# ucsdarclab/diffco

Measured on AMD Instinct MI355X. Metric: million collision-score+grad evals/sec, 7-DoF FK-kernel, 2k supports, higher is better.
Workload: dtype f32

## Files before the change

diffco_amd/csrc/score_kernel.h:

```cpp
#pragma once
#include <hip/hip_runtime.h>
#include <type_traits>
#include <stdint.h>
#include "fk_device.h"

namespace dcx {

enum { KF_RQ2 = 0,
       KF_POLY1 = 1,
       KF_GEN = 2 };

enum { MODE_SCORE = 0,
       MODE_GRAD_ROW = 1,
       MODE_GRAD_UP = 2 };

struct ScoreArgs {
    const float* rows;
    const float* centre;
    const FkProg* fk;
    const float* q;
    const float* upstream;
    float* score;
    float* grad;
    int64_t B;
// ... 117 lines not shown
#endif
#define DCX_D2_ACCS(D) (!DCX_D2_MULTI ? 1 : (D) >= 32 ? 4 : (D) >= 16 ? 2 : 1)
#ifndef DCX_PAIR2
#define DCX_PAIR2 1
#endif
#ifndef DCX_PAIR2_MAX_D
#define DCX_PAIR2_MAX_D 8
#endif
#ifndef DCX_PAIR2_LOADS
#define DCX_PAIR2_LOADS 1
#endif
#ifndef DCX_LOAD_GROUPS
#define DCX_LOAD_GROUPS 1
#endif

template <int KF, bool CLAMPED = false>
__device__ __forceinline__ void kernel_eval(float d2, const ScoreArgs& a, float& val, float& g) {
    if constexpr (KF == KF_RQ2) {
        const float t = fmaf(0.5f * a.kp0, d2, 1.0f);
        const float u = __builtin_amdgcn_rcpf(t);
        val = u * u;
        g = (-2.0f * a.kp0) * (val * u);
    } else if constexpr (KF == KF_POLY1) {
        const float d2c = CLAMPED ? d2 : fmaxf(d2, 1e-30f);
        const float ri = __builtin_amdgcn_rsqf(d2c);
        val = d2c * ri;
        g = ri;
    } else {
        if (a.kind == DCX_K_RQ) {
            const float p = a.kp1;
            const float t = fmaf(a.kp0 / p, d2, 1.0f);
            val = powf(t, -p);
            g = (-2.0f * a.kp0) * val * __builtin_amdgcn_rcpf(t);
        } else if (a.kind == DCX_K_POLY) {
            const int k = (int)a.kp0;
            const float ie = 1.0f / a.kp1;
            const float d2c = fmaxf(d2, 1e-30f);
            const float ri = __builtin_amdgcn_rsqf(d2c);
            const float r = d2c * ri;
            float rk2 = (k >= 2) ? 1.0f : ri;
            for (int i = 2; i < k; ++i) rk2 *= r;
            if (k & 1) {
                val = rk2 * d2c * ie;
                g = (float)k * rk2 * ie;
            } else {
                const float lg = 0.5f * logf(d2c);
                val = rk2 * d2c * lg * ie;
                g = rk2 * fmaf((float)k, lg, 1.0f) * ie;
            }
        } else {
            const float ie2 = 1.0f / (a.kp0 * a.kp0);
            const float v2 = fmaf(d2, ie2, 1.0f);
            const float rv = __builtin_amdgcn_rsqf(v2);
            val = v2 * rv;
            g = rv * ie2;
        }
    }
}

template <int KF>
__device__ __forceinline__ float d2_seed(const ScoreArgs& a) {
    if constexpr (KF == KF_RQ2) return a.kp0;
    else return 0.0f;
}
template <int KF>
inline constexpr float kGradScale = (KF == KF_RQ2) ? -4.0f : 1.0f;
template <int KF, bool CLAMPED = false>
__device__ __forceinline__ void sweep_eval(float t, const ScoreArgs& a, float& val, float& g) {
    if constexpr (KF == KF_RQ2) {
        const float u = __builtin_amdgcn_rcpf(t);
        val = u * u;
        g = val * u;
    } else {
        kernel_eval<KF, CLAMPED>(t, a, val, g);
    }
}

struct LdsPlan {
    int fk, q, x, g, f, red, total;
};
__host__ __device__ inline LdsPlan lds_plan(int dof, int d_fk, int frame_floats, int red_slots, int acc_floats,
                                            bool alias_xg = false) {
    LdsPlan p;
    p.x = 0;
    p.g = alias_xg ? p.x : p.x + 64 * d_fk;
    p.red = p.x;
    const int end_xg = p.g + 64 * d_fk;
    const int end_red = p.red + (red_slots < 1 ? 1 : red_slots) * acc_floats * 64;
    p.q = end_xg > end_red ? end_xg : end_red;
    p.f = p.q + ((64 * dof + 3) & ~3);
    p.fk = p.f + 64 * frame_floats;
    p.total = p.fk;
    return p;
}

#ifndef DCX_MINW_SLACK
#define DCX_MINW_SLACK 0
#endif
constexpr int sweep_min_waves(int D, int CC, int KF, bool QT = false) {
    if (QT) return 4;
    const int need = 3 * D + 2 * CC + 16 + DCX_MINW_SLACK + (KF == 2 ? 40 : 0);
    return need <= 64 ? 8 : need <= 72 ? 7 : need <= 80 ? 6 : need <= 96 ? 5 : need <= 128 ? 4 : need <= 168 ? 3 : need <= 256 ? 2 : 1;
}

__device__ __forceinline__ int fresh_lane() {
    int l = (int)__builtin_amdgcn_mbcnt_hi(~0u, __builtin_amdgcn_mbcnt_lo(~0u, 0u));
    asm volatile("" : "+v"(l));
    return l;
}

template <class Args>
__device__ __forceinline__ const __attribute__((address_space(4))) Args& reload_kernargs() {
    auto p = (const __attribute__((address_space(4))) Args*)__builtin_amdgcn_kernarg_segment_ptr();
    asm volatile("" : "+s"(p));
    return *p;
}
__device__ __forceinline__ const __attribute__((address_space(4))) ScoreArgs& reload_args() { return reload_kernargs<ScoreArgs>(); }
#define DCX_COPY_DH(dst, src)          \
    do {                               \
        (dst).prog = (src).prog;       \
        (dst).n_dwords = (src).n_dwords; \
        (dst).n_steps = (src).n_steps; \
        (dst).end0 = (src).end0;       \
        (dst).n_chains = (src).n_chains; \
        (dst).pt = (src).pt;           \
        (dst).bare = (src).bare;       \
        (dst).real = (src).real;       \
        (dst).n_pt = (src).n_pt;       \
        (dst).shared_q = (src).shared_q; \
    } while (0)

__device__ __forceinline__ void row_opaque(float& u, float& v) { asm volatile("" : "+v"(u), "+v"(v)); }

#ifndef DCX_XF_TAU
#define DCX_XF_TAU 0.01f
#endif
#ifndef DCX_XF_FLUSH
#define DCX_XF_FLUSH 64
#endif

constexpr bool xf_applies(int D, int CC, int KF) {
    const int used = D + CC + (CC > 1 ? 1 : 0);
    const int parts = (4 * used <= (CC > 1 ? DCX_P0_MAX_MULTI : DCX_P0_MAX_SINGLE)) ? 0 : (used + 37) / 38;
    return (KF == KF_POLY1 || KF == KF_RQ2) && used + 1 <= 38 && parts <= 1;
}
constexpr bool spare_applies(int D, int CC, int KF) {
    return CC == 1 && (D % 4) == 0 && D >= 4 && D <= 12 && (KF == KF_POLY1 || KF == KF_RQ2) && D + 4 <= (D + 2 + 3) / 4 * 4;
}
constexpr bool p2_applies(int D, int CC, int KF) {
    return DCX_PAIR2 && DCX_PAIR2_LOADS && CC == 1 && (D % 2) == 0 && D <= DCX_PAIR2_MAX_D && 4 * (D + 1) <= DCX_P0_MAX_SINGLE &&
           (KF == KF_RQ2 || KF == KF_POLY1);
}

template <int D, int KF, int CC, int MODE, bool XF = false, int NACC = 0, bool NS = false, bool SP = false>
__device__ __forceinline__ void sweep_rows(const ScoreArgs& a, const float (&x_in)[D], const float (&up)[CC], int j0, int j1,
                                           float (&sc)[CC], float (&gx)[D]) {
    static_assert(!NS || (CC > 1 && MODE == MODE_GRAD_UP), "NS: the gradient sweep of a multi-class model");
    static_assert(!SP || (XF && spare_applies(D, CC, KF) && xf_applies(D, CC, KF)), "the spare form: expanded, one class, D = 4, 8, 12");
    float x[D];
    float e_sp = 0.0f, tot_sp = 0.0f;
    int col_sp = 0;
    if constexpr (SP) {
        const int c = a.spare - 1;
        e_sp = x_in[D - 1];
#pragma unroll
        for (int k = 0; k + 1 < D; ++k) {
            e_sp = (k == c) ? x_in[k] : e_sp;
            x[k] = (k == c) ? x_in[D - 1] : x_in[k];
        }
        x[D - 1] = 0.0f;
        col_sp = c;
        asm volatile("" : "+v"(col_sp));
    } else {
#pragma unroll
        for (int k = 0; k < D; ++k) x[k] = x_in[k];
    }
    using L = RowLayout<D, CC>;
    constexpr bool GRAD = (MODE != MODE_SCORE);
    v2f gx2[D / 2 + 1];
#pragma unroll
    for (int k = 0; k < D / 2 + 1; ++k) gx2[k] = v2f{0.0f, 0.0f};
    cfloat_ptr rows = (cfloat_ptr)(uintptr_t)a.rows;
    if constexpr (SP) {
        uint64_t rp = (uint64_t)(uintptr_t)a.rows;
        asm volatile("" : "+s"(rp));
        rows = (cfloat_ptr)(uintptr_t)rp;
    }
    constexpr int USED_DIRECT = D + CC + (CC > 1 ? 1 : 0);
    constexpr bool XFA = XF && xf_applies(D, CC, KF);
    constexpr int USED = SP ? D + 4 : USED_DIRECT + (XFA ? 1 : 0);
    constexpr int RSTRIDE = L::RS;
    constexpr int PARTS = SP ? 0 : (4 * USED <= (CC > 1 ? DCX_P0_MAX_MULTI : DCX_P0_MAX_SINGLE)) ? 0 : (USED + 37) / 38;
    constexpr bool SC2 = (CC > 1 && PARTS == 1);
    v2f sc2[CC / 2 + 1];
#pragma unroll
    for (int i = 0; i < CC / 2 + 1; ++i) sc2[i] = v2f{0.0f, 0.0f};
    auto add_scores = [&](auto weight_of, float val) __attribute__((always_inline)) {
        if constexpr (NS) {
            (void)val;
        } else if constexpr (SC2) {
            const v2f v2 = {val, val};
#pragma unroll
            for (int c = 0; c + 1 < CC; c += 2) sc2[c / 2] = __builtin_elementwise_fma(v2f{weight_of(c), weight_of(c + 1)}, v2, sc2[c / 2]);
            if constexpr (CC & 1) sc[CC - 1] = fmaf(weight_of(CC - 1), val, sc[CC - 1]);
#pragma unroll
            for (int c = 0; c + 1 < CC; c += 2) asm volatile("" : "+v"(sc2[c / 2]));
            if constexpr (CC & 1) asm volatile("" : "+v"(sc[CC - 1]));
        } else {
#pragma unroll
            for (int c = 0; c < CC; ++c) sc[c] = fmaf(weight_of(c), val, sc[c]);
        }
    };

    v2f xm[D / 2 + 1], ga[D / 2 + 1];
    float xm_tail = 0.0f, ga_tail = 0.0f, xx = 0.0f, thr = 1e-30f, asum = 0.0f;
    if constexpr (XFA) {
#pragma unroll
        for (int k = 0; k < D; ++k) xx = fmaf(x[k], x[k], xx);
        if constexpr (SP) xx = fmaf(e_sp, e_sp, xx);
        thr = fmaxf(DCX_XF_TAU * xx, 1e-30f);
#pragma unroll
        for (int k = 0; k + 1 < D; k += 2) {
            xm[k / 2] = v2f{-2.0f * x[k], -2.0f * x[k + 1]};
            ga[k / 2] = v2f{0.0f, 0.0f};
        }
        if constexpr (D & 1) xm_tail = -2.0f * x[D - 1];
        if constexpr (SP) xm[D / 2 - 1].y = 1.0f;
    }
    auto d2_x = [&](const auto& r) __attribute__((always_inline)) -> float {
        constexpr int NA = NACC > 0 ? NACC : DCX_D2_ACCS(D);
        v2f acc[NA];
        if constexpr (SP) acc[0] = v2f{xx, 0.0f};
        else acc[0] = v2f{xx + r[L::SS_OFF], 0.0f};
#pragma unroll
        for (int i = 1; i < NA; ++i) acc[i] = v2f{0.0f, 0.0f};
#pragma unroll
        for (int k = 0; k + 1 < D; k += 2) {
            const v2f rv = {r[k], r[k + 1]};
            acc[(k / 2) % NA] = __builtin_elementwise_fma(xm[k / 2], rv, acc[(k / 2) % NA]);
        }
#pragma unroll
        for (int i = 1; i < NA; ++i) acc[0] += acc[i];
        float d2 = acc[0].x + acc[0].y;
        if constexpr (D & 1) d2 = fmaf(xm_tail, r[D - 1], d2);
        if constexpr (KF == KF_POLY1) return fmaxf(d2, thr);
        else return d2;
    };
    auto coef_of = [&](const auto& r, float g) __attribute__((always_inline)) -> float {
        if constexpr (MODE == MODE_GRAD_ROW) {
            return g * r[CC > 1 ? L::WSUM_OFF : L::W_OFF];
        } else {
            float wb = 0.0f;
#pragma unroll
            for (int c = 0; c < CC; ++c) wb = fmaf(up[c], r[L::W_OFF + c], wb);
            return g * wb;
        }
    };
    auto apply_x = [&](const auto& r, float d2c, auto sign, bool keep) __attribute__((always_inline)) {
        constexpr int SIGN = decltype(sign)::value;
        float val, g;
        sweep_eval<KF, true>(d2c, a, val, g);
        if constexpr (PARTS == 1) row_opaque(val, g);
        constexpr bool SCORE_BY_COEF = (KF == KF_POLY1 && CC == 1 && MODE == MODE_GRAD_ROW);
        if constexpr (!SCORE_BY_COEF) {
            if constexpr (SIGN < 0) val = keep ? -val : 0.0f;
            add_scores([&](int c) __attribute__((always_inline)) { return r[L::W_OFF + c]; }, val);
        }
        if constexpr (GRAD) {
            float coef = coef_of(r, g);
            if constexpr (PARTS == 1) asm volatile("" : "+v"(coef));
            if constexpr (SIGN < 0) coef = keep ? -coef : 0.0f;
            if constexpr (SCORE_BY_COEF) sc[0] = fmaf(coef, d2c, sc[0]);
            const v2f c2 = {coef, coef};
#pragma unroll
            for (int k = 0; k + 1 < D; k += 2) {
                v2f rv = {r[k], r[k + 1]};
                if constexpr (SP) {
                    if (k == D - 2) rv = v2f{r[D + 2], r[D + 3]};
                }
                ga[k / 2] = __builtin_elementwise_fma(c2, rv, ga[k / 2]);
            }
            if constexpr (D & 1) ga_tail = fmaf(coef, r[D - 1], ga_tail);
            if constexpr (!SP) asum += coef;
        }
    };
    auto pair_x = [&](const auto& r) __attribute__((always_inline)) -> float {
        const float d2 = d2_x(r);
        apply_x(r, d2, std::integral_constant<int, 1>{}, true);
        return d2;
    };
    auto fix_near = [&](const auto& r, float d2c) __attribute__((always_inline)) {
        const bool nr = d2c <= thr;
        apply_x(r, d2c, std::integral_constant<int, -1>{}, nr);
        const v2f mh = {-0.5f, -0.5f};
        v2f dacc = {0.0f, 0.0f};
#pragma unroll
        for (int k = 0; k + 1 < D; k += 2) {
            const v2f rv = {r[k], r[k + 1]};
            v2f dk = xm[k / 2] * mh - rv;
            if constexpr (SP) {
                if (k == D - 2) dk.y = e_sp;
            }
            dacc = __builtin_elementwise_fma(dk, dk, dacc);
        }
        float d2d = dacc.x + dacc.y;
        if constexpr (D & 1) {
            const float dl_tail = -0.5f * xm_tail - r[D - 1];
            d2d = fmaf(dl_tail, dl_tail, d2d);
        }
        float val, g;
        kernel_eval<KF>(d2d, a, val, g);
        if constexpr (SP && KF == KF_POLY1) val = (d2d == d2d) ? val : d2d;
        val = nr ? val : 0.0f;
        if constexpr (!NS) {
#pragma unroll
// ... 338 lines not shown
            cfloat_ptr r = rows + (size_t)j * RSTRIDE + P0;
#ifdef DCX_EXP_NO_LOADS
            if (exp_real_loads <= 2) {
#pragma unroll
                for (int e = 0; e < LEN; ++e) asm volatile("" : "+s"(dst[e]));
                return;
            }
            --exp_real_loads;
#endif
#pragma unroll
            for (int e = 0; e < LEN; ++e) dst[e] = r[e];
        };
        auto consume = [&](const float (&b)[PS], auto pc) __attribute__((always_inline)) {
            if constexpr (XFA) {
                single_x(b);
                return;
            }
            constexpr int P0 = decltype(pc)::value * PS;
            constexpr int LEN = (USED - P0 < PS) ? (USED - P0) : PS;
            if constexpr (decltype(pc)::value == 0) {
                acc[0] = v2f{d2_seed<KF>(a), 0.0f};
#pragma unroll
                for (int i = 1; i < NA; ++i) acc[i] = v2f{0.0f, 0.0f};
            }
#pragma unroll
            for (int e = 0; e < LEN; ++e) {
                const int g = P0 + e;
                if (g + 1 < D && (g & 1) == 0) {
                    const v2f xv = {x[g], x[g + 1]};
                    const v2f rv = {b[e], b[e + 1]};
                    dp[g / 2] = xv - rv;
                    acc[(g / 2) % NA] = __builtin_elementwise_fma(dp[g / 2], dp[g / 2], acc[(g / 2) % NA]);
                } else if (g == D - 1 && (D & 1)) {
                    tail_d = x[g] - b[e];
                } else if (g >= D && g < D + CC) {
                    wv[g - D] = b[e];
                } else if (CC > 1 && g == D + CC) {
                    wsum = b[e];
                }
            }
            if constexpr (decltype(pc)::value == PARTS - 1) {
#pragma unroll
                for (int i = 1; i < NA; ++i) acc[0] += acc[i];
                float d2 = acc[0].x + acc[0].y;
                if constexpr (D & 1) d2 = fmaf(tail_d, tail_d, d2);
                float val, g;
                sweep_eval<KF>(d2, a, val, g);
                if constexpr (PARTS == 1) row_opaque(val, g);
                add_scores([&](int c) __attribute__((always_inline)) { return wv[c]; }, val);
                if constexpr (GRAD) {
                    float coef;
                    if constexpr (MODE == MODE_GRAD_ROW) {
                        coef = g * (CC > 1 ? wsum : wv[0]);
                    } else {
                        float wb = 0.0f;
#pragma unroll
                        for (int c = 0; c < CC; ++c) wb = fmaf(up[c], wv[c], wb);
                        coef = g * wb;
                    }
                    if constexpr (PARTS == 1) asm volatile("" : "+v"(coef));
                    const v2f c2 = {coef, coef};
#pragma unroll
                    for (int k = 0; k + 1 < D; k += 2) gx2[k / 2] = __builtin_elementwise_fma(c2, dp[k / 2], gx2[k / 2]);
                    if constexpr (D & 1) gx[D - 1] = fmaf(coef, tail_d, gx[D - 1]);
                }
            }
        };
        using P0c = std::integral_constant<int, 0>;
        using P1c = std::integral_constant<int, PARTS - 1>;
        if (j0 < j1) {
            const int jl = j1 - 1;
            if constexpr (PARTS == 1) {
                static_assert(PS <= RSTRIDE, "a whole row in groups of four floats stays inside its stride");
                load_part(bufA, j0, P0c{});
                int j = j0;
                for (; j + 1 < j1; j += 2) {
                    __builtin_amdgcn_s_waitcnt(0xC07F);
                    __builtin_amdgcn_sched_barrier(0);
                    load_part(bufB, j + 1, P0c{});
                    __builtin_amdgcn_sched_barrier(0);
                    consume(bufA, P0c{});
                    __builtin_amdgcn_sched_barrier(0);
                    __builtin_amdgcn_s_waitcnt(0xC07F);
                    __builtin_amdgcn_sched_barrier(0);
                    load_part(bufA, (j + 2 < j1) ? j + 2 : jl, P0c{});
                    __builtin_amdgcn_sched_barrier(0);
                    consume(bufB, P0c{});
                    __builtin_amdgcn_sched_barrier(0);
                    if constexpr (XFA && GRAD) {
                        if ((j & (DCX_XF_FLUSH - 2)) == 0) flush_x();
                    }
                }
                if (j < j1) consume(bufA, P0c{});
            } else if constexpr (PARTS == 2) {
                load_part(bufA, j0, P0c{});
                for (int j = j0; j < j1; ++j) {
                    __builtin_amdgcn_s_waitcnt(0xC07F);
                    __builtin_amdgcn_sched_barrier(0);
                    load_part(bufB, j, P1c{});
                    __builtin_amdgcn_sched_barrier(0);
                    consume(bufA, P0c{});
                    __builtin_amdgcn_sched_barrier(0);
                    __builtin_amdgcn_s_waitcnt(0xC07F);
                    __builtin_amdgcn_sched_barrier(0);
                    load_part(bufA, (j + 1 < j1) ? j + 1 : jl, P0c{});
                    __builtin_amdgcn_sched_barrier(0);
                    consume(bufB, P1c{});
                    __builtin_amdgcn_sched_barrier(0);
                }
            } else {
                auto step = [&](auto self, auto uc, int j) __attribute__((always_inline)) -> void {
                    constexpr int U = decltype(uc)::value;
                    constexpr int NU = U + 1;
                    __builtin_amdgcn_s_waitcnt(0xC07F);
                    __builtin_amdgcn_sched_barrier(0);
                    {
                        const int jr = j + NU / PARTS;
                        const int row = jr < j1 ? jr : jl;
                        if constexpr (NU % 2 == 0) load_part(bufA, row, std::integral_constant<int, NU % PARTS>{});
                        else load_part(bufB, row, std::integral_constant<int, NU % PARTS>{});
                    }
                    __builtin_amdgcn_sched_barrier(0);
                    if constexpr (U % 2 == 0) consume(bufA, std::integral_constant<int, U % PARTS>{});
                    else consume(bufB, std::integral_constant<int, U % PARTS>{});
                    __builtin_amdgcn_sched_barrier(0);
                    if constexpr (U + 1 < 2 * PARTS) self(self, std::integral_constant<int, U + 1>{}, j);
                };
                load_part(bufA, j0, P0c{});
                int j = j0;
                for (; j + 1 < j1; j += 2) step(step, P0c{}, j);
                if (j < j1) {
                    auto tail = [&](auto self, auto pc) __attribute__((always_inline)) -> void {
                        constexpr int P = decltype(pc)::value;
                        __builtin_amdgcn_s_waitcnt(0xC07F);
                        __builtin_amdgcn_sched_barrier(0);
                        if constexpr (P + 1 < PARTS) {
                            if constexpr ((P + 1) % 2 == 0) load_part(bufA, j, std::integral_constant<int, P + 1>{});
                            else load_part(bufB, j, std::integral_constant<int, P + 1>{});
                        }
                        __builtin_amdgcn_sched_barrier(0);
                        if constexpr (P % 2 == 0) consume(bufA, pc);
                        else consume(bufB, pc);
                        __builtin_amdgcn_sched_barrier(0);
                        if constexpr (P + 1 < PARTS) self(self, std::integral_constant<int, P + 1>{});
                    };
                    tail(tail, P0c{});
                }
            }
        }
    }

    if constexpr (XFA && GRAD) {
        flush_x();
        if constexpr (SP) {
            const int c = __builtin_amdgcn_readfirstlane(col_sp);
            const float gl = e_sp * tot_sp;
            float gsw = gl;
#pragma unroll
            for (int k = 0; k + 1 < D; ++k) {
                const float h = (k & 1) ? ga[k / 2].y : ga[k / 2].x;
                gsw = (k == c) ? -h : gsw;
                gx[k] += (k == c) ? gl : -h;
            }
            gx[D - 1] += gsw;
        } else {
#pragma unroll
        for (int k = 0; k + 1 < D; k += 2) {
            gx[k] -= ga[k / 2].x;
            gx[k + 1] -= ga[k / 2].y;
        }
        if constexpr (D & 1) gx[D - 1] -= ga_tail;
        }
    } else {
#pragma unroll
        for (int k = 0; k + 1 < D; k += 2) {
            gx[k] += gx2[k / 2].x;
            gx[k + 1] += gx2[k / 2].y;
        }
        if constexpr (P2) {
            sc[0] += scp.x + scp.y;
            if constexpr (GRAD) {
#pragma unroll
                for (int k = 0; k < D; ++k) gx[k] += gp[k].x + gp[k].y;
            }
        }
    }
    if constexpr (SC2) {
#pragma unroll
        for (int c = 0; c + 1 < CC; c += 2) {
            sc[c] += sc2[c / 2].x;
            sc[c + 1] += sc2[c / 2].y;
        }
    }
    if constexpr (GRAD && kGradScale<KF> != 1.0f) {
#pragma unroll
        for (int k = 0; k < D; ++k) gx[k] *= kGradScale<KF>;
    }
}

constexpr int kQtSlices = 4;
constexpr bool qt_applies(int D, int CC, int KF, int MODE) {
    return (D == 12 || D == 24) && CC == 1 && (MODE == 1  || MODE == 0 ) && KF != 2 ;
}
template <int D, int KF, bool GRAD>
__device__ __forceinline__ void sweep_rows_lds(const ScoreArgs& a, const float (&x)[D], const float* slice, int per, float& sc0,
                                               float (&gx)[D]) {
    static_assert(D % 4 == 0, "rows are read as whole float4s");
    using L = RowLayout<D, 1>;
    v2f g2[D / 2];
#pragma unroll
    for (int k = 0; k < D / 2; ++k) g2[k] = v2f{0.0f, 0.0f};
    typedef float v4f_t __attribute__((ext_vector_type(4)));
    auto load_row = [&](float (&r)[D + 1], int jj) __attribute__((always_inline)) {
        const float* p = slice + (size_t)jj * L::RS;
#pragma unroll
        for (int q = 0; q < D / 4; ++q) {
            const v4f_t v = *reinterpret_cast<const v4f_t*>(p + 4 * q);
            r[4 * q] = v.x; r[4 * q + 1] = v.y; r[4 * q + 2] = v.z; r[4 * q + 3] = v.w;
        }
        r[D] = p[L::W_OFF];
    };
    auto pair = [&](const float (&r)[D + 1]) __attribute__((always_inline)) {
        v2f dp[D / 2];
        constexpr int NA = DCX_D2_ACCS(D);
        v2f acc[NA];
        acc[0] = v2f{d2_seed<KF>(a), 0.0f};
#pragma unroll
        for (int i = 1; i < NA; ++i) acc[i] = v2f{0.0f, 0.0f};
#pragma unroll
        for (int k = 0; k + 1 < D; k += 2) {
            const v2f xv = {x[k], x[k + 1]};
            const v2f rv = {r[k], r[k + 1]};
            dp[k / 2] = xv - rv;
            acc[(k / 2) % NA] = __builtin_elementwise_fma(dp[k / 2], dp[k / 2], acc[(k / 2) % NA]);
        }
#pragma unroll
        for (int i = 1; i < NA; ++i) acc[0] += acc[i];
        const float d2 = acc[0].x + acc[0].y;
        float val, g;
        sweep_eval<KF>(d2, a, val, g);
        sc0 = fmaf(r[D], val, sc0);
        if constexpr (GRAD) {
            const float coef = g * r[D];
            const v2f c2 = {coef, coef};
#pragma unroll
            for (int k = 0; k + 1 < D; k += 2) g2[k / 2] = __builtin_elementwise_fma(c2, dp[k / 2], g2[k / 2]);
        }
    };
    float ra[D + 1], rb[D + 1];
    load_row(ra, 0);
    int jj = 0;
    for (; jj + 2 <= per; jj += 2) {
        load_row(rb, jj + 1);
        pair(ra);
        load_row(ra, jj + 2 < per ? jj + 2 : jj + 1);
        pair(rb);
    }
    if (jj < per) pair(ra);
    if constexpr (GRAD) {
#pragma unroll
        for (int k = 0; k + 1 < D; k += 2) {
            gx[k] += g2[k / 2].x * kGradScale<KF>;
            gx[k + 1] += g2[k / 2].y * kGradScale<KF>;
        }
    }
}

template <int ACC, int E0 = 0, int E1 = ACC>
__device__ __forceinline__ void fold_partial_rows(float* sRed, int wave, int lane, int nw) {
    auto fold_rows = [&](auto nwc) __attribute__((always_inline)) {
        constexpr int NWC = decltype(nwc)::value;
        for (int e = E0 + wave; e < E1; e += NWC) {
            float r[NWC];
#pragma unroll
            for (int w = 0; w < NWC; ++w) r[w] = sRed[((size_t)w * ACC + e) * 64 + lane];
            float v = r[0];
#pragma unroll
            for (int w = 1; w < NWC; ++w) v += r[w];
            sRed[e * 64 + lane] = v;
        }
    };
    if (nw == 16) fold_rows(std::integral_constant<int, 16>{});
    else if (nw == 8) fold_rows(std::integral_constant<int, 8>{});
    else if (nw == 4) fold_rows(std::integral_constant<int, 4>{});
    else if (nw == 2) fold_rows(std::integral_constant<int, 2>{});
    else {
        for (int e = E0 + wave; e < E1; e += nw) {
            float v = sRed[e * 64 + lane];
            for (int w = 1; w < nw; ++w) v += sRed[((size_t)w * ACC + e) * 64 + lane];
            sRed[e * 64 + lane] = v;
        }
    }
}


template <int D, int KF, int CC, int MODE, int MAXT, bool XF, bool QT, bool SP>
__device__ __forceinline__ void score_body(const ScoreArgs& a) {
    extern __shared__ __attribute__((aligned(16))) float smem[];
    constexpr bool GRAD = (MODE != MODE_SCORE);
    constexpr int ACC = (GRAD ? D : 0) + CC;
    constexpr int TILE = QT ? 16 : 64;
    static_assert(!QT || (!XF && qt_applies(D, CC, KF, MODE)), "the quarter tile: direct form, one class, row weights");

    int lane = threadIdx.x & 63;
    const int wave = __builtin_amdgcn_readfirstlane(threadIdx.x >> 6);
    const int nw = blockDim.x >> 6;
    const int64_t b0 = (int64_t)blockIdx.x * TILE;
    const int nb = (int)((a.B - b0) < TILE ? (a.B - b0) : TILE);
    const int dof = a.dof;
    const LdsPlan lp = lds_plan(dof, a.d_fk, a.frame_floats, nw > 1 ? a.red_slots : 0, ACC, true);
    float* sQ = smem + lp.q;
    float* sX = smem + lp.x;
    float* sF = smem + lp.f;

    auto stage_rows = [&](int first_wave, int row0, int row1) __attribute__((always_inline)) {
        if constexpr (QT) {
            constexpr int RS4 = RowLayout<D, CC>::RS / 4;
            typedef float v4f_t __attribute__((ext_vector_type(4)));
            const v4f_t* src = reinterpret_cast<const v4f_t*>(a.rows);
            constexpr int RSQ = RowLayout<D, CC>::RS;
            const int p0 = a.qt_per_g[0], p1 = a.qt_per_g[1], p2 = a.qt_per_g[2], p3 = a.qt_per_g[3];
            const int r1 = 16 * p0, r2 = r1 + 16 * p1, r3 = r2 + 16 * p2;
            const int b1 = 16 * (p0 * RSQ + 4), b2 = b1 + 16 * (p1 * RSQ + 4), b3 = b2 + 16 * (p2 * RSQ + 4);
            float* dst = smem + a.qt_off;
            for (int e = row0 * RS4 + (int)threadIdx.x - 64 * first_wave; e < row1 * RS4; e += (int)blockDim.x - 64 * first_wave) {
                const int row = e / RS4, q4 = e - row * RS4;
                const int g = (row >= r3) ? 3 : (row >= r2) ? 2 : (row >= r1) ? 1 : 0;
                const int per = (g == 3) ? p3 : (g == 2) ? p2 : (g == 1) ? p1 : p0;
                const int rr = row - ((g == 3) ? r3 : (g == 2) ? r2 : (g == 1) ? r1 : 0);
                const int base = (g == 3) ? b3 : (g == 2) ? b2 : (g == 1) ? b1 : 0;
                const int sl = per > 0 ? rr / per : 0, jj = rr - sl * per;
                v4f_t v = {0.0f, 0.0f, 0.0f, 0.0f};
                if (row < a.S) v = src[(size_t)row * RS4 + q4];
                if (per > 0 && sl < 16) *reinterpret_cast<v4f_t*>(dst + base + sl * (per * RSQ + 4) + jj * RSQ + 4 * q4) = v;
            }
        }
    };
    DCX_TS(0);
    DCX_TSB(0);
    const FkWalk fw = fk_stage_sel(a.fkk, a.fk, a.fk_dwords, a.dh, smem + lp.fk, threadIdx.x, blockDim.x);
#ifdef DCX_TIMING
    if (threadIdx.x == 0) dcx_fk_ts = (a.ts && blockIdx.x == a.ts_block && blockIdx.y == 0) ? a.ts : nullptr;
#endif
    {
        const float* qsrc = a.q + b0 * dof;
        const int n = nb * dof;
        if constexpr (QT) {
            for (int i = threadIdx.x; i < 64 * dof; i += blockDim.x) {
                const int c = (i / dof) & 15;
                sQ[i] = qsrc[(c < nb ? c : nb - 1) * dof + (i % dof)];
            }
            stage_rows(0, 0, a.qt_front);
        } else {
            for (int i = threadIdx.x; i < 64 * dof; i += blockDim.x) sQ[i] = qsrc[i < n ? i : (i % dof) + (nb - 1) * dof];
        }
    }
    __syncthreads();
    DCX_TS(1);
    fk_trig_sel(fw, a.dh, sQ + lane * dof, sF + lane, wave, nw);
    __syncthreads();
    DCX_TS(6);
    if (a.fkk == 2 && a.jt_rows) {
        dh2_chain_rows_sel(fw.dh, a.dh, sX + lane, sF + lane, wave);
        if (QT && wave >= 2 * a.dh.n_chains) stage_rows(2 * a.dh.n_chains, a.qt_front, kQtSlices * nw * a.qt_per);
    } else if (wave == 0) {
        fk_chain_sel(fw, a.dh, sQ + lane * dof, sX + lane, sF + lane);
    } else {
        stage_rows(1, a.qt_front, kQtSlices * nw * a.qt_per);
    }
    __syncthreads();

    DCX_TS(2);
    float x[D];
    if (a.d_fk == D) {
#pragma unroll
        for (int k = 0; k < D; ++k) x[k] = sX[k * 64 + lane];
    } else {
#pragma unroll
        for (int k = 0; k < D; ++k) x[k] = (k < a.d_fk) ? sX[k * 64 + lane] : 0.0f;
    }
    if constexpr (XF) {
        cfloat_ptr cen = (cfloat_ptr)(uintptr_t)a.centre;
#pragma unroll
        for (int k = 0; k < D; ++k) x[k] -= cen[k];
    }
    if (nw > 1) __syncthreads();

    float up[CC];
    if constexpr (MODE == MODE_GRAD_UP) {
        const int64_t bl = b0 + (lane < nb ? lane : nb - 1);
        const int hot = (a.nz > 1) ? (int)blockIdx.z : a.one_hot;
#pragma unroll
        for (int c = 0; c < CC; ++c) up[c] = (hot >= 0) ? (c == hot ? 1.0f : 0.0f) : (c < a.c_out ? a.upstream[bl * a.c_out + c] : 0.0f);
        if (a.hinge == 2) {
#pragma unroll
            for (int c = 0; c < CC; ++c) up[c] = (c < a.c_out && up[c] - a.hinge_margin_c[c < 8 ? c : 7] > 0.0f) ? a.hinge_weight : 0.0f;
        }
    }

    float sc[CC];
    float gx[D];
#pragma unroll
    for (int c = 0; c < CC; ++c) sc[c] = 0.0f;
#pragma unroll
    for (int k = 0; k < D; ++k) gx[k] = 0.0f;
    const int ybase = blockIdx.y * a.s_super;
    const int yend = (ybase + a.s_super < a.S) ? (ybase + a.s_super) : a.S;
    int j0, j1;
    wave_slice(wave, nw, a.s_chunk, a.s_skew, ybase, yend, j0, j1);

    DCX_TSB(1);
    if constexpr (QT) {
        constexpr int RSQ = RowLayout<D, CC>::RS;
        const int g = wave >> 2;
        const int per = a.qt_per_g[g];
        int base = 0;
        for (int h = 0; h < g; ++h) base += 16 * (a.qt_per_g[h] * RSQ + 4);
        const float* slice = smem + a.qt_off + base + ((wave & 3) * kQtSlices + (lane >> 4)) * (per * RSQ + 4);
        sweep_rows_lds<D, KF, GRAD>(a, x, slice, per, sc[0], gx);
    } else {
        sweep_rows<D, KF, CC, MODE, XF, 0, false, SP>(a, x, up, j0, j1, sc, gx);
    }
    DCX_TS(3);
    {
    const auto& b = reload_args();
    int lane = fresh_lane();
    const int wave = __builtin_amdgcn_readfirstlane(threadIdx.x >> 6);
    const int nw = blockDim.x >> 6;
    const int64_t b0 = (int64_t)blockIdx.x * TILE;
    const size_t tile = (size_t)blockIdx.x * gridDim.z + blockIdx.z;
    const int nb = (int)((b.B - b0) < TILE ? (b.B - b0) : TILE);
    const int dof = b.dof;
    const LdsPlan lp = lds_plan(dof, b.d_fk, b.frame_floats, nw > 1 ? b.red_slots : 0, ACC, true);
    float* sQ = smem + lp.q;
    float* sG = smem + lp.g;
    float* sF = smem + lp.f;
    float* sRed = smem + lp.red;
    DhArgs dhb;
    DCX_COPY_DH(dhb, b.dh);
    FkWalk fw;
    fw.fkk = b.fkk;
    fw.g = b.fk;
    fw.fk = (fk_cptr)(uintptr_t)(uint32_t)(uintptr_t)(smem + lp.fk);
    fw.dh = (dh_cptr)(uintptr_t)(uint32_t)(uintptr_t)(smem + lp.fk);
    const bool split = b.partial != nullptr;
    const bool par_tail = nw > 1 && b.red_slots != 1 && (!split || b.tile_done != nullptr);
    bool r1_done = false;
    if constexpr (QT && GRAD) {
        if (b.jt_waves && b.qt_scr > 0) {
            r1_done = true;
            dh2_vjp_r1_sel(fw.dh, dhb, sF + lane, smem + b.qt_scr + lane, wave);
        }
    }
    if (par_tail) {
        float* mine = sRed + (size_t)wave * ACC * 64 + lane;
#pragma unroll
        for (int c = 0; c < CC; ++c) mine[c * 64] = sc[c];
        if constexpr (GRAD) {
#pragma unroll
            for (int k = 0; k < D; ++k) mine[(CC + k) * 64] = gx[k];
        }
        __syncthreads();
        DCX_TS(16);
        const bool opoll = split && b.pwords != nullptr;
        const bool publisher = opoll && blockIdx.y != 0;
        unsigned long long* wout = opoll ? b.pwords + ((tile * b.ys + blockIdx.y) * ACC) * 64 + lane : nullptr;
        float* out = (split && !opoll) ? b.partial + (tile * b.ys + blockIdx.y) * ACC * 64 + lane : nullptr;
        auto fold_mine = [&](auto nwc) __attribute__((always_inline)) {
            constexpr int NWC = decltype(nwc)::value;
            const int nwr = NWC > 0 ? NWC : nw;
            for (int e = wave; e < ACC; e += nwr) {
                float v;
                if constexpr (NWC > 0) {
                    float r[NWC];
#pragma unroll
                    for (int w = 0; w < NWC; ++w) r[w] = sRed[((size_t)w * ACC + e) * 64 + lane];
                    v = r[0];
#pragma unroll
                    for (int w = 1; w < NWC; ++w) v += r[w];
                } else {
                    v = sRed[e * 64 + lane];
                    for (int w = 1; w < nw; ++w) v += sRed[((size_t)w * ACC + e) * 64 + lane];
                }
                if constexpr (QT) {
                    v += __shfl_xor(v, 16, 64);
                    v += __shfl_xor(v, 32, 64);
                }
                if (publisher) __hip_atomic_store(wout + e * 64, ((unsigned long long)b.ptag << 32) | (unsigned long long)__float_as_uint(v), __ATOMIC_RELAXED, __HIP_MEMORY_SCOPE_AGENT);
                else if (split && !opoll) __hip_atomic_store(out + e * 64, v, __ATOMIC_RELAXED, __HIP_MEMORY_SCOPE_AGENT);
                else sRed[e * 64 + lane] = v;
            }
        };
        if (nw == 16) fold_mine(std::integral_constant<int, 16>{});
        else if (nw == 8) fold_mine(std::integral_constant<int, 8>{});
        else if (nw == 4) fold_mine(std::integral_constant<int, 4>{});
        else if (nw == 2) fold_mine(std::integral_constant<int, 2>{});
        else fold_mine(std::integral_constant<int, 0>{});
        DCX_TS(17);
        if (opoll) {
            if (publisher) return;
            __syncthreads();
            const bool jt_here = GRAD && b.jt_waves;
            r1_done = jt_here && nw >= 2 + 2 * dhb.n_chains;
            if (r1_done && wave >= 2) dh2_vjp_r1_sel(fw.dh, dhb, sF + lane, sRed + (size_t)ACC * 64 + lane, wave - 2);
            const unsigned long long* wtile = b.pwords + (tile * b.ys) * ACC * 64 + lane;
            for (int e = wave; e < ACC; e += nw) {
                float tot = 0.0f;
                int spins = 0;
                for (;;) {
                    tot = sRed[e * 64 + lane];
                    bool all = true;
                    for (int y = 1; y < b.ys; y += 8) {
                        unsigned long long wv[8];
#pragma unroll
                        for (int v = 0; v < 8; ++v)
                            if (y + v < b.ys) wv[v] = __hip_atomic_load(wtile + ((size_t)(y + v) * ACC + e) * 64, __ATOMIC_RELAXED, __HIP_MEMORY_SCOPE_AGENT);
#pragma unroll
                        for (int v = 0; v < 8; ++v)
                            if (y + v < b.ys) {
                                all = all && ((unsigned int)(wv[v] >> 32) == b.ptag);
                                tot += __uint_as_float((unsigned int)wv[v]);
                            }
                    }
                    if (__builtin_amdgcn_ballot_w64(!all) == 0) break;
                    if (++spins > (1 << 21)) {
                        tot = __builtin_nanf("");
                        if (lane == 0) __hip_atomic_store(b.giveup, 1, __ATOMIC_RELAXED, __HIP_MEMORY_SCOPE_SYSTEM);
                        break;
                    }
                    __builtin_amdgcn_s_sleep(1);
                }
                for (int y = 1; y < b.ys; ++y)
                    __hip_atomic_store(const_cast<unsigned long long*>(wtile) + ((size_t)y * ACC + e) * 64, 0ull, __ATOMIC_RELAXED, __HIP_MEMORY_SCOPE_AGENT);
                sRed[e * 64 + lane] = tot;
            }
            DCX_FK_TS(11, 2);
        } else if (split) {
#ifdef DCX_HANDOVER_FENCE
            __builtin_amdgcn_fence(__ATOMIC_RELEASE, "agent");
#else
#if defined(__HIP_DEVICE_COMPILE__) && !defined(__gfx950__) && !defined(__gfx942__)
#error "the drained write-through hand-over relies on gfx942 / gfx950 lowering (agent-scope atomic store = global_store sc1, counted by vmcnt): build other targets with -DDCX_HANDOVER_FENCE"
#endif
            asm volatile("s_waitcnt vmcnt(0)" ::: "memory");
#endif
            __syncthreads();
            DCX_FK_TS(8, 2);
            const bool jt_here = GRAD && b.jt_waves;
            unsigned int* flag = reinterpret_cast<unsigned int*>(sRed + ((size_t)ACC + (jt_here ? 12 * dhb.n_pt : 0)) * 64);
            r1_done = jt_here && nw >= 2 + 2 * dhb.n_chains;
            if (wave == 0) {
                if (lane == 0) *flag = __hip_atomic_fetch_add(b.tile_done + tile * kCounterStride, 1u, __ATOMIC_RELAXED, __HIP_MEMORY_SCOPE_AGENT);
            } else if (r1_done) {
                dh2_vjp_r1_sel(fw.dh, dhb, sF + lane, sRed + (size_t)ACC * 64 + lane, wave - 2);
            }
            __syncthreads();
            const unsigned int arrived = __builtin_amdgcn_readfirstlane(*flag);
            DCX_FK_TS(9, 2);
            if (arrived != (unsigned int)b.ys - 1u) return;
            if (wave == 0 && lane == 0) b.tile_done[tile * kCounterStride] = 0u;
            asm volatile("" ::: "memory");
            const float* part = b.partial + tile * b.ys * ACC * 64 + lane;
            for (int e = wave; e < ACC; e += nw) {
                float tot = 0.0f;
                for (int y = 0; y < b.ys; y += 8) {
                    float r[8];
#pragma unroll
                    for (int v = 0; v < 8; ++v)
                        if (y + v < b.ys) r[v] = __hip_atomic_load(part + ((size_t)(y + v) * ACC + e) * 64, __ATOMIC_RELAXED, __HIP_MEMORY_SCOPE_AGENT);
#pragma unroll
                    for (int v = 0; v < 8; ++v)
                        if (y + v < b.ys) tot += r[v];
                }
                sRed[e * 64 + lane] = tot;
            }
            DCX_FK_TS(11, 2);
        }
        __syncthreads();
        DCX_TS(4);
        if (wave == 0 && b.score != nullptr && lane < nb && blockIdx.z == 0) {
#pragma unroll
            for (int c = 0; c < CC; ++c)
                if (c < b.c_out) b.score[(b0 + lane) * b.c_out + c] = sRed[c * 64 + lane];
        }
        if constexpr (!GRAD) {
            return;
        } else {
            if (b.jt_waves) {
                float scale = 1.0f;
                if constexpr (CC == 1 && MODE == MODE_GRAD_ROW) {
                    if (b.upstream != nullptr) scale = b.upstream[b0 + (lane < nb ? lane : nb - 1)];
                    if (b.hinge) scale = (sRed[lane] - b.hinge_margin > 0.0f) ? b.hinge_weight : 0.0f;
                }
                float* gq = smem + lp.q;
                float* scr = (QT && r1_done) ? smem + b.qt_scr + lane : sRed + (size_t)ACC * 64 + lane;
                if (!r1_done) {
                    dh2_vjp_r1_sel(fw.dh, dhb, sF + lane, scr, wave);
                    __syncthreads();
                }
                dh2_vjp_r1b(fw.dh, dhb, sRed + CC * 64 + lane, scale, scr, gq + lane * dof, dof, wave, nw);
                __syncthreads();
                dh2_vjp_r2_sel(fw.dh, dhb, sF + lane, scr, gq + lane * dof, wave);
                if (dhb.n_chains > 1 && !dhb.shared_q) __syncthreads();
                if (wave != 0) return;
                DCX_TS(5);
                __builtin_amdgcn_fence(__ATOMIC_ACQ_REL, "workgroup");
                __builtin_amdgcn_wave_barrier();
                float* gdst = b.grad + b0 * b.grad_stride + (b.nz > 1 ? (size_t)blockIdx.z * dof : 0);
                const int n = nb * dof;
                if (b.grad_stride == dof) {
                    for (int i = lane; i < n; i += 64) gdst[i] = gq[i];
                } else {
                    for (int i = lane; i < n; i += 64) gdst[(int64_t)(i / dof) * b.grad_stride + (i % dof)] = gq[i];
                }
                DCX_TSB(3);
                return;
            }
            if (wave != 0) return;
#pragma unroll
            for (int c = 0; c < CC; ++c) sc[c] = sRed[c * 64 + lane];
#pragma unroll
            for (int k = 0; k < D; ++k) gx[k] = sRed[(CC + k) * 64 + lane];
        }
    } else {
    if (nw > 1 && b.red_slots == 1) {
        for (int w = 1; w < nw; ++w) {
            if (wave == w) {
#pragma unroll
                for (int c = 0; c < CC; ++c) sRed[c * 64 + lane] = sc[c];
                if constexpr (GRAD) {
#pragma unroll
                    for (int k = 0; k < D; ++k) sRed[(CC + k) * 64 + lane] = gx[k];
                }
            }
            __syncthreads();
            if (wave == 0) {
#pragma unroll
                for (int c = 0; c < CC; ++c) sc[c] += sRed[c * 64 + lane];
                if constexpr (GRAD) {
#pragma unroll
                    for (int k = 0; k < D; ++k) gx[k] += sRed[(CC + k) * 64 + lane];
                }
            }
            __syncthreads();
        }
        if (wave != 0) return;
    } else if (nw > 1) {
        float* mine = sRed + (size_t)wave * ACC * 64 + lane;
#pragma unroll
        for (int c = 0; c < CC; ++c) mine[c * 64] = sc[c];
        if constexpr (GRAD) {
#pragma unroll
            for (int k = 0; k < D; ++k) mine[(CC + k) * 64] = gx[k];
        }
        __syncthreads();
        fold_partial_rows<ACC>(sRed, wave, lane, nw);
        __syncthreads();
        if (wave != 0) return;
#pragma unroll
        for (int c = 0; c < CC; ++c) sc[c] = sRed[c * 64 + lane];
        if constexpr (GRAD) {
#pragma unroll
            for (int k = 0; k < D; ++k) gx[k] = sRed[(CC + k) * 64 + lane];
        }
    }

    DCX_TS(4);
    if (__builtin_expect(b.partial != nullptr, 0)) {
        float* out = b.partial + (tile * b.ys + blockIdx.y) * ACC * 64 + lane;
        if (b.tile_done == nullptr) {
#pragma unroll
            for (int c = 0; c < CC; ++c) out[c * 64] = sc[c];
            if constexpr (GRAD) {
#pragma unroll
                for (int k = 0; k < D; ++k) out[(CC + k) * 64] = gx[k];
            }
            return;
        }
#pragma unroll
        for (int c = 0; c < CC; ++c) __hip_atomic_store(out + c * 64, sc[c], __ATOMIC_RELAXED, __HIP_MEMORY_SCOPE_AGENT);
        if constexpr (GRAD) {
#pragma unroll
            for (int k = 0; k < D; ++k)
                __hip_atomic_store(out + (CC + k) * 64, gx[k], __ATOMIC_RELAXED, __HIP_MEMORY_SCOPE_AGENT);
        }
#ifdef DCX_HANDOVER_FENCE
        __builtin_amdgcn_fence(__ATOMIC_RELEASE, "agent");
#else
        asm volatile("s_waitcnt vmcnt(0)" ::: "memory");
#endif
        unsigned int arrived = 0;
        if (lane == 0) arrived = __hip_atomic_fetch_add(b.tile_done + tile * kCounterStride, 1u, __ATOMIC_RELAXED, __HIP_MEMORY_SCOPE_AGENT);
        arrived = __builtin_amdgcn_readfirstlane(arrived);
        if (arrived != (unsigned int)b.ys - 1u) return;
        if (lane == 0) b.tile_done[tile * kCounterStride] = 0u;
        asm volatile("" ::: "memory");
        const float* part = b.partial + tile * b.ys * ACC * 64 + lane;
#pragma unroll 1
        for (int e0 = 0; e0 < ACC; e0 += 4) {
            float tot[4];
#pragma unroll
            for (int u = 0; u < 4; ++u) tot[u] = 0.0f;
#pragma unroll 1
            for (int y = 0; y < b.ys; y += 4) {
                float r[4][4];
#pragma unroll
                for (int v = 0; v < 4; ++v) {
                    const int yy = (y + v < b.ys) ? y + v : y;
#pragma unroll
                    for (int u = 0; u < 4; ++u) {
                        const int e = (e0 + u < ACC) ? e0 + u : ACC - 1;
                        r[v][u] = __hip_atomic_load(part + ((size_t)yy * ACC + e) * 64, __ATOMIC_RELAXED, __HIP_MEMORY_SCOPE_AGENT);
                    }
                }
#pragma unroll
                for (int v = 0; v < 4; ++v) {
                    if (y + v < b.ys) {
#pragma unroll
                        for (int u = 0; u < 4; ++u) tot[u] += r[v][u];
                    }
                }
            }
#pragma unroll
            for (int u = 0; u < 4; ++u)
                if (e0 + u < ACC) sRed[(e0 + u) * 64 + lane] = tot[u];
        }
#pragma unroll
        for (int c = 0; c < CC; ++c) sc[c] = sRed[c * 64 + lane];
        if constexpr (GRAD) {
#pragma unroll
            for (int k = 0; k < D; ++k) gx[k] = sRed[(CC + k) * 64 + lane];
        }
    }

    if (b.score != nullptr && lane < nb && blockIdx.z == 0) {
#pragma unroll
        for (int c = 0; c < CC; ++c)
            if (c < b.c_out) b.score[(b0 + lane) * b.c_out + c] = sc[c];
    }
    }

    if constexpr (GRAD) {
        float scale = 1.0f;
        if constexpr (CC == 1 && MODE == MODE_GRAD_ROW) {
            if (b.upstream != nullptr) scale = b.upstream[b0 + (lane < nb ? lane : nb - 1)];
            if (b.hinge) scale = (sc[0] - b.hinge_margin > 0.0f) ? b.hinge_weight : 0.0f;
        }
        if (b.d_fk == D) {
#pragma unroll
            for (int k = 0; k < D; ++k) sG[k * 64 + lane] = gx[k] * scale;
        } else {
#pragma unroll
            for (int k = 0; k < D; ++k)
                if (k < b.d_fk) sG[k * 64 + lane] = gx[k] * scale;
        }
        DCX_FK_TS(12, 2);
        float* gq = smem + lp.q;
        fk_vjp_sel(fw, dhb, sQ + lane * dof, sF + lane, sG + lane, gq + lane * dof, dof);
        DCX_TS(5);
        __builtin_amdgcn_fence(__ATOMIC_ACQ_REL, "workgroup");
        __builtin_amdgcn_wave_barrier();
        float* gdst = b.grad + b0 * b.grad_stride + (b.nz > 1 ? (size_t)blockIdx.z * dof : 0);
        const int n = nb * dof;
        if (b.grad_stride == dof) {
            for (int i = lane; i < n; i += 64) gdst[i] = gq[i];
        } else {
            for (int i = lane; i < n; i += 64) gdst[(int64_t)(i / dof) * b.grad_stride + (i % dof)] = gq[i];
        }
        DCX_TSB(3);
    }
    }
}

template <int D, int KF, int CC, int MODE, int MAXT, bool XF = false, bool QT = false>
__global__ __launch_bounds__(MAXT, sweep_min_waves(D, CC, KF, QT)) void score_kernel(const ScoreArgs a) {
    score_body<D, KF, CC, MODE, MAXT, XF, QT, false>(a);
}
template <int D, int KF, int CC, int MODE, int MAXT>
__global__ __launch_bounds__(MAXT, sweep_min_waves(D, CC, KF, false)) void score_kernel_sp(const ScoreArgs a) {
    static_assert(spare_applies(D, CC, KF), "no spare form for this shape");
    score_body<D, KF, CC, MODE, MAXT, true, false, true>(a);
}

struct FinishArgs {
    const float* partial;
    const FkProg* fk;
    const float* q;
    const float* upstream;
    float* score;
    float* grad;
    int64_t B;
    int64_t grad_stride;
    int32_t ys, acc, C, Dt, dof, d_fk, frame_floats, want_grad;
    int32_t c_out;
    int32_t hinge;
    float hinge_margin, hinge_weight;
};

}
```

Baseline: 808.3.

## Pre-stage centred, spare-swapped features in LDS before the spare-form sweep

For the spare-form path, the feature centring and the spare-column swap are done once, cooperatively across waves in LDS, before the sweep. The sweep then reads features in a fixed order with no per-lane selects. The swapped gradient slot is undone at the output, partial-store and cross-wave fold stages. This removes the per-thread select chains from the sweep prologue and epilogue. In exchange it adds an extra barrier, extra LDS traffic, and index remapping in the reduction paths.

After: 823.5 (median of 6 runs). 1.9% higher.

```diff
diff --git a/diffco_amd/csrc/score_kernel.h b/diffco_amd/csrc/score_kernel.h
--- a/diffco_amd/csrc/score_kernel.h
+++ b/diffco_amd/csrc/score_kernel.h
@@ -293,15 +293,21 @@
            (KF == KF_RQ2 || KF == KF_POLY1);
 }
 
-template <int D, int KF, int CC, int MODE, bool XF = false, int NACC = 0, bool NS = false, bool SP = false>
+template <int D, int KF, int CC, int MODE, bool XF = false, int NACC = 0, bool NS = false, bool SP = false, bool PRE = false>
 __device__ __forceinline__ void sweep_rows(const ScoreArgs& a, const float (&x_in)[D], const float (&up)[CC], int j0, int j1,
                                            float (&sc)[CC], float (&gx)[D]) {
     static_assert(!NS || (CC > 1 && MODE == MODE_GRAD_UP), "NS: the gradient sweep of a multi-class model");
     static_assert(!SP || (XF && spare_applies(D, CC, KF) && xf_applies(D, CC, KF)), "the spare form: expanded, one class, D = 4, 8, 12");
+    static_assert(!PRE || SP, "pre-staged features: the spare form only");
     float x[D];
     float e_sp = 0.0f, tot_sp = 0.0f;
     int col_sp = 0;
-    if constexpr (SP) {
+    if constexpr (PRE) {
+        e_sp = x_in[D - 1];
+#pragma unroll
+        for (int k = 0; k + 1 < D; ++k) x[k] = x_in[k];
+        x[D - 1] = 0.0f;
+    } else if constexpr (SP) {
         const int c = a.spare - 1;
         e_sp = x_in[D - 1];
 #pragma unroll
@@ -946,7 +952,12 @@
 
     if constexpr (XFA && GRAD) {
         flush_x();
-        if constexpr (SP) {
+        if constexpr (PRE) {
+            const float gl = e_sp * tot_sp;
+#pragma unroll
+            for (int k = 0; k + 1 < D; ++k) gx[k] += -((k & 1) ? ga[k / 2].y : ga[k / 2].x);
+            gx[D - 1] += gl;
+        } else if constexpr (SP) {
             const int c = __builtin_amdgcn_readfirstlane(col_sp);
             const float gl = e_sp * tot_sp;
             float gsw = gl;
@@ -1165,15 +1176,36 @@
     __syncthreads();
 
     DCX_TS(2);
+    if constexpr (SP) {
+        cfloat_ptr cen = (cfloat_ptr)(uintptr_t)a.centre;
+        const int dfk = a.d_fk;
+        const int c = (dfk == D) ? a.spare - 1 : D - 1;
+        for (int k = wave; k < dfk; k += nw) {
+            if (k == D - 1 && c != D - 1) continue;
+            const float u = sX[k * 64 + lane] - cen[k];
+            if (k == c && c != D - 1) {
+                const float v = sX[(D - 1) * 64 + lane] - cen[D - 1];
+                sX[k * 64 + lane] = v;
+                sX[(D - 1) * 64 + lane] = u;
+            } else {
+                sX[k * 64 + lane] = u;
+            }
+        }
+        if (nw > 1) __syncthreads();
+    }
     float x[D];
     if (a.d_fk == D) {
 #pragma unroll
         for (int k = 0; k < D; ++k) x[k] = sX[k * 64 + lane];
+    } else if constexpr (SP) {
+        cfloat_ptr cen = (cfloat_ptr)(uintptr_t)a.centre;
+#pragma unroll
+        for (int k = 0; k < D; ++k) x[k] = (k < a.d_fk) ? sX[k * 64 + lane] : 0.0f - cen[k];
     } else {
 #pragma unroll
         for (int k = 0; k < D; ++k) x[k] = (k < a.d_fk) ? sX[k * 64 + lane] : 0.0f;
     }
-    if constexpr (XF) {
+    if constexpr (XF && !SP) {
         cfloat_ptr cen = (cfloat_ptr)(uintptr_t)a.centre;
 #pragma unroll
         for (int k = 0; k < D; ++k) x[k] -= cen[k];
@@ -1213,7 +1245,7 @@
         const float* slice = smem + a.qt_off + base + ((wave & 3) * kQtSlices + (lane >> 4)) * (per * RSQ + 4);
         sweep_rows_lds<D, KF, GRAD>(a, x, slice, per, sc[0], gx);
     } else {
-        sweep_rows<D, KF, CC, MODE, XF, 0, false, SP>(a, x, up, j0, j1, sc, gx);
+        sweep_rows<D, KF, CC, MODE, XF, 0, false, SP, SP>(a, x, up, j0, j1, sc, gx);
     }
     DCX_TS(3);
     {
@@ -1240,6 +1272,8 @@
     const bool split = b.partial != nullptr;
     const bool par_tail = nw > 1 && b.red_slots != 1 && (!split || b.tile_done != nullptr);
     bool r1_done = false;
+    int sp_cs = D - 1;
+    auto sp_slot = [&](int k) __attribute__((always_inline)) -> int { return (k == sp_cs) ? D - 1 : (k == D - 1) ? sp_cs : k; };
     if constexpr (QT && GRAD) {
         if (b.jt_waves && b.qt_scr > 0) {
             r1_done = true;
@@ -1285,11 +1319,56 @@
                 else sRed[e * 64 + lane] = v;
             }
         };
+        auto fold_mine_sp = [&](auto nwc) __attribute__((always_inline)) {
+            constexpr int NWC = decltype(nwc)::value;
+            const int nwr = NWC > 0 ? NWC : nw;
+            const int csw = (b.d_fk == D) ? b.spare - 1 : D - 1;
+            auto fold_one = [&](int e) __attribute__((always_inline)) -> float {
+                float v;
+                if constexpr (NWC > 0) {
+                    float r[NWC > 0 ? NWC : 1];
+#pragma unroll
+                    for (int w = 0; w < NWC; ++w) r[w] = sRed[((size_t)w * ACC + e) * 64 + lane];
+                    v = r[0];
+#pragma unroll
+                    for (int w = 1; w < NWC; ++w) v += r[w];
+                } else {
+                    v = sRed[e * 64 + lane];
+                    for (int w = 1; w < nw; ++w) v += sRed[((size_t)w * ACC + e) * 64 + lane];
+                }
+                return v;
+            };
+            auto put = [&](int e, float v) __attribute__((always_inline)) {
+                if (publisher) __hip_atomic_store(wout + e * 64, ((unsigned long long)b.ptag << 32) | (unsigned long long)__float_as_uint(v), __ATOMIC_RELAXED, __HIP_MEMORY_SCOPE_AGENT);
+                else if (split && !opoll) __hip_atomic_store(out + e * 64, v, __ATOMIC_RELAXED, __HIP_MEMORY_SCOPE_AGENT);
+                else sRed[e * 64 + lane] = v;
+            };
+            const int e_ex = (csw != D - 1) ? CC + csw : -1, e_skip = (csw != D - 1) ? CC + D - 1 : -1;
+            for (int e = wave; e < ACC; e += nwr) {
+                if (e == e_skip) continue;
+                if (e == e_ex) {
+                    const float vc = fold_one(CC + D - 1);
+                    const float vl = fold_one(e);
+                    put(e, vc);
+                    put(CC + D - 1, vl);
+                } else {
+                    put(e, fold_one(e));
+                }
+            }
+        };
+        if constexpr (SP && GRAD) {
+            if (nw == 16) fold_mine_sp(std::integral_constant<int, 16>{});
+            else if (nw == 8) fold_mine_sp(std::integral_constant<int, 8>{});
+            else if (nw == 4) fold_mine_sp(std::integral_constant<int, 4>{});
+            else if (nw == 2) fold_mine_sp(std::integral_constant<int, 2>{});
+            else fold_mine_sp(std::integral_constant<int, 0>{});
+        } else {
         if (nw == 16) fold_mine(std::integral_constant<int, 16>{});
         else if (nw == 8) fold_mine(std::integral_constant<int, 8>{});
         else if (nw == 4) fold_mine(std::integral_constant<int, 4>{});
         else if (nw == 2) fold_mine(std::integral_constant<int, 2>{});
         else fold_mine(std::integral_constant<int, 0>{});
+        }
         DCX_TS(17);
         if (opoll) {
             if (publisher) return;
@@ -1417,6 +1496,7 @@
             for (int k = 0; k < D; ++k) gx[k] = sRed[(CC + k) * 64 + lane];
         }
     } else {
+    if constexpr (SP && GRAD) sp_cs = (b.d_fk == D) ? b.spare - 1 : D - 1;
     if (nw > 1 && b.red_slots == 1) {
         for (int w = 1; w < nw; ++w) {
             if (wave == w) {
@@ -1465,7 +1545,10 @@
         if (b.tile_done == nullptr) {
 #pragma unroll
             for (int c = 0; c < CC; ++c) out[c * 64] = sc[c];
-            if constexpr (GRAD) {
+            if constexpr (SP && GRAD) {
+#pragma unroll
+                for (int k = 0; k < D; ++k) out[(CC + sp_slot(k)) * 64] = gx[k];
+            } else if constexpr (GRAD) {
 #pragma unroll
                 for (int k = 0; k < D; ++k) out[(CC + k) * 64] = gx[k];
             }
@@ -1473,7 +1556,12 @@
         }
 #pragma unroll
         for (int c = 0; c < CC; ++c) __hip_atomic_store(out + c * 64, sc[c], __ATOMIC_RELAXED, __HIP_MEMORY_SCOPE_AGENT);
-        if constexpr (GRAD) {
+        if constexpr (SP && GRAD) {
+#pragma unroll
+            for (int k = 0; k < D; ++k)
+                __hip_atomic_store(out + (CC + sp_slot(k)) * 64, gx[k], __ATOMIC_RELAXED, __HIP_MEMORY_SCOPE_AGENT);
+            sp_cs = D - 1;
+        } else if constexpr (GRAD) {
 #pragma unroll
             for (int k = 0; k < D; ++k)
                 __hip_atomic_store(out + (CC + k) * 64, gx[k], __ATOMIC_RELAXED, __HIP_MEMORY_SCOPE_AGENT);
@@ -1540,7 +1628,11 @@
             if (b.upstream != nullptr) scale = b.upstream[b0 + (lane < nb ? lane : nb - 1)];
             if (b.hinge) scale = (sc[0] - b.hinge_margin > 0.0f) ? b.hinge_weight : 0.0f;
         }
-        if (b.d_fk == D) {
+        if constexpr (SP) {
+#pragma unroll
+            for (int k = 0; k < D; ++k)
+                if (k < b.d_fk) sG[sp_slot(k) * 64 + lane] = gx[k] * scale;
+        } else if (b.d_fk == D) {
 #pragma unroll
             for (int k = 0; k < D; ++k) sG[k * 64 + lane] = gx[k] * scale;
         } else {
```
